# GPUs/goVideoCompressor

Hardware: AMD Instinct MI355X
Metric: encoded frames/sec (whole node), 1080p30->H.264 CRF23 (higher is better)
Workload: dtype uint8 (8-bit 4:2:0 samples, int32 transforms)

## Files before the change

csrc/kernels/bindings_hip.cc:

```cpp
#include <pybind11/pybind11.h>
#include <pybind11/stl.h>

#include <cstdint>
#include <stdexcept>
#include <vector>

#include "../common/hevc_ctu_coder.h"
#include "hevc_decode.h"
#include "route.h"

namespace py = pybind11;

extern "C" {
long long mivc_hevc_entropy_state_bytes(int W, int H);
int mivc_launch_hevc_entropy(const void* pic, int B, const int* qp, const void* ctu, const void* cu, const void* col,
                             const unsigned long long* nzmap, const int16_t* cy, const int16_t* cb, const int16_t* cr,
                             uint8_t* state, long long state_bytes, uint8_t* out, unsigned cap, unsigned* sizes,
                             int* errs, unsigned long long* offs, unsigned long long* offs_host, uint8_t* dst,
                             unsigned long long dst_cap, int* overflow, void* stream, unsigned long long* prof,
                             int* gprog, void* gctx);
int mivc_launch_hevc_decode(const mivc::gpu::HevcDecParams* p, int stage, void* stream);
void mivc_launch_synth(void* y, void* u, void* v, int width, int height, int slots, int frames, int frame0,
                       uint32_t seed, int bit_depth, int slot0, void* stream, int kind);
void mivc_launch_prep(const uint8_t* in_y, const uint8_t* in_u, const uint8_t* in_v, int w, int h,
                      int64_t in_stride_y, int64_t in_stride_c, int nframes, uint8_t* out_y, uint8_t* out_u,
                      uint8_t* out_v, int ow, int oh, int W, int H, void* stream, const int* fsel);
void mivc_launch_rgb_to_i420(const uint8_t* rgb, int w, int h, int nframes, uint8_t* y, uint8_t* u, uint8_t* v,
                             void* stream);
void mivc_launch_me(int B, int wmb, int hmb, const uint8_t* src_y, const uint8_t* ref_y, const int16_t* pred_mv,
                    int16_t* out_mv, int* out_cost, uint8_t* out_pred, int* out_intra_cost, const int* qp, int range,
                    int subpel, uint8_t* hp, const int8_t* aq, int planes_ready, int early_sad, void* stream,
                    const int* gate_cost, int gate_thresh, const int16_t* cost_mv, const void* route, int nbuf,
                    int role, int want, const int16_t* seed_mv);
void mivc_launch_me_ref_select(int B, int wmb, int hmb, int nref, int16_t* mv, int16_t* mv8, int* cost, uint8_t* pred,
                               const int16_t* xmv, const int* xcost, const uint8_t* xpred, int8_t* mref, const int* qp,
                               const int8_t* aq, void* stream, const void* route);
void mivc_launch_b_spatial(int B, int wmb, int hmb, void* hdr, const void* col, const uint8_t* src, const uint8_t* ref1,
                           const uint8_t* hp1, const uint8_t* const* ref0k, const uint8_t* const* hp0k, const int* w1,
                           int nref, uint8_t* pred_out, int* err, void* stream, const int* intra_cost, int* cost,
                           const int* qp, const int8_t* aq, int bias, const void* route, int nbuf);
void mivc_launch_b_direct(int B, int wmb, int hmb, const void* col, const int* dsf, const int* direct_copy, int nref,
                          int16_t* dmv, int8_t* dref, int16_t* pm0, int16_t* pm1, void* stream, const void* route,
                          int nbuf, uint8_t* czero, const int8_t* cmap);
void mivc_launch_b_spatial_exact(int B, int wmb, int hmb, void* hdr, const int* intra_cost, const int* cost,
                                 const uint8_t* czero, uint8_t* fix, void* stream, const void* route, int slice_rows,
                                 int tol);
void mivc_launch_b_spatial_fixup(int B, int wmb, int hmb, const void* hdr, const uint8_t* fix, const uint8_t* ref0,
                                 const uint8_t* hp0, const uint8_t* ref1, const uint8_t* hp1, uint8_t* pred_out,
                                 void* stream, const void* route, int nbuf);
void mivc_launch_p_refine(int B, int wmb, int hmb, const uint8_t* src_y, const uint8_t* ref, const uint8_t* hp,
                          const int16_t* mv_in, int16_t* mv_out, int* cost, const int16_t* pm, uint8_t* pred,
                          const int* qp, const int8_t* aq, void* stream, const void* route, int nbuf,
                          const uint8_t* chg_in, uint8_t* chg_out);
void mivc_launch_b_decide(int B, int wmb, int hmb, const uint8_t* src_y, const uint8_t* ref0, const uint8_t* ref1,
                          const uint8_t* hp0, const uint8_t* hp1, const int16_t* mv0, const int16_t* mv1,
                          const int* cost0, const int* cost1, const uint8_t* pred0, const uint8_t* pred1,
                          const int16_t* pm0, const int16_t* pm1, const int16_t* dmv, const int* qp, const int8_t* aq,
                          void* hdr, uint8_t* pred_out, int* cost_out, void* stream, const int* w1, int nref,
                          const int8_t* dref, const uint8_t* const* ref0k, const uint8_t* const* hp0k,
                          int direct_only, int bparts, int have_direct, int spatial, int dbias, const void* route,
                          int nbuf, const uint8_t* czero);
void mivc_launch_aq_offsets(int B, int wmb, int hmb, const uint8_t* sy, const uint8_t* su, const uint8_t* sv,
                            float strength, const float* extra, long long extra_stride, int8_t* out, void* stream,
                            const void* route);
void mivc_launch_mbtree(int B, int F, int lbw, int lbh, const int* blk_cost, const int* blk_mv, void* prop,
                        float strength, float* out, void* stream);
// ... 143 lines not shown
}

PYBIND11_MODULE(_hip, m) {
  m.doc() = "govideocompressor_amd gfx950 kernels (raw-pointer launch shims)";
  m.attr("arch") = "gfx950";
  m.def("route_bytes", []() { return static_cast<int>(sizeof(mivc::gpu::SlotRoute)); });

  m.def("synth", [](uintptr_t y, uintptr_t u, uintptr_t v, int w, int h, int slots, int frames, int frame0,
                    uint32_t seed, uintptr_t stream, int bit_depth, int slot0, int kind) {
    if (bit_depth != 8 && bit_depth != 10) throw std::invalid_argument("synth: bit_depth must be 8 or 10");
    if (kind < 0 || kind > 6) throw std::invalid_argument("synth: content kind 0..6");
    mivc_launch_synth(P<void>(y), P<void>(u), P<void>(v), w, h, slots, frames, frame0, seed, bit_depth, slot0,
                      S(stream), kind);
  }, py::arg("y"), py::arg("u"), py::arg("v"), py::arg("w"), py::arg("h"), py::arg("slots"), py::arg("frames"),
     py::arg("frame0"), py::arg("seed"), py::arg("stream"), py::arg("bit_depth") = 8, py::arg("slot0") = 0,
     py::arg("kind") = 0);
  m.def("prep", [](uintptr_t iy, uintptr_t iu, uintptr_t iv, int w, int h, int64_t sy, int64_t sc, int n,
                   uintptr_t oy, uintptr_t ou, uintptr_t ov, int ow, int oh, int W, int H, uintptr_t stream,
                   uintptr_t fsel) {
    if (ow != w || oh != h) throw std::invalid_argument("prep: resample with ops.scale (scale.hip) first");
    if (W < w || H < h || w < 2 || h < 2) throw std::invalid_argument("prep: bad geometry");
    mivc_launch_prep(P<uint8_t>(iy), P<uint8_t>(iu), P<uint8_t>(iv), w, h, sy, sc, n, P<uint8_t>(oy), P<uint8_t>(ou),
                     P<uint8_t>(ov), ow, oh, W, H, S(stream), P<int>(fsel));
  }, py::arg("iy"), py::arg("iu"), py::arg("iv"), py::arg("w"), py::arg("h"), py::arg("sy"), py::arg("sc"), py::arg("n"),
     py::arg("oy"), py::arg("ou"), py::arg("ov"), py::arg("ow"), py::arg("oh"), py::arg("W"), py::arg("H"),
     py::arg("stream"), py::arg("fsel") = 0);
  m.def("rgb_to_i420", [](uintptr_t rgb, int w, int h, int n, uintptr_t y, uintptr_t u, uintptr_t v,
                          uintptr_t stream) {
    mivc_launch_rgb_to_i420(P<uint8_t>(rgb), w, h, n, P<uint8_t>(y), P<uint8_t>(u), P<uint8_t>(v), S(stream));
  });
  m.def("me", [](int B, int wmb, int hmb, uintptr_t src, uintptr_t ref, uintptr_t pred_mv, uintptr_t out_mv,
                 uintptr_t out_cost, uintptr_t out_pred, uintptr_t out_intra, uintptr_t qp, int range, int subpel,
                 uintptr_t stream, uintptr_t hp, uintptr_t aq, int planes_ready, int early_sad, uintptr_t gate_cost,
                 int gate_thresh, uintptr_t cost_mv, uintptr_t route, int nbuf, int role, int want, uintptr_t seed_mv) {
    if (planes_ready && !hp) throw std::invalid_argument("me: planes_ready needs the hp buffer");
    if (route && (nbuf < 1 || role < 0 || role > 4 || (want != 0 && want != 1) || !planes_ready))
      throw std::invalid_argument("me: a routed search needs nbuf, a role (list-0 0..3 / list-1 4), want P/B and the planes");
    mivc_launch_me(B, wmb, hmb, P<uint8_t>(src), P<uint8_t>(ref), P<int16_t>(pred_mv), P<int16_t>(out_mv),
                   P<int>(out_cost), P<uint8_t>(out_pred), P<int>(out_intra), P<int>(qp), range, subpel,
                   P<uint8_t>(hp), P<int8_t>(aq), planes_ready, early_sad, S(stream), P<int>(gate_cost), gate_thresh,
                   P<int16_t>(cost_mv), P<void>(route), nbuf, role, want, P<int16_t>(seed_mv));
  }, py::arg("B"), py::arg("wmb"), py::arg("hmb"), py::arg("src"), py::arg("ref"), py::arg("pred_mv"),
     py::arg("out_mv"), py::arg("out_cost"), py::arg("out_pred"), py::arg("out_intra"), py::arg("qp"),
     py::arg("range"), py::arg("subpel"), py::arg("stream"), py::arg("hp") = 0, py::arg("aq") = 0,
     py::arg("planes_ready") = 0, py::arg("early_sad") = 0, py::arg("gate_cost") = 0, py::arg("gate_thresh") = 0,
     py::arg("cost_mv") = 0, py::arg("route") = 0, py::arg("nbuf") = 0, py::arg("role") = 0, py::arg("want") = 0,
     py::arg("seed_mv") = 0);
  m.def("me_ref_select", [](int B, int wmb, int hmb, int nref, uintptr_t mv, uintptr_t mv8, uintptr_t cost,
                            uintptr_t pred, uintptr_t xmv, uintptr_t xcost, uintptr_t xpred, uintptr_t mref,
                            uintptr_t qp, uintptr_t aq, uintptr_t stream, uintptr_t route) {
    if (nref < 2 || nref > 4) throw std::invalid_argument("me_ref_select: nref in 2..4");
    mivc_launch_me_ref_select(B, wmb, hmb, nref, P<int16_t>(mv), P<int16_t>(mv8), P<int>(cost), P<uint8_t>(pred),
                              P<int16_t>(xmv), P<int>(xcost), P<uint8_t>(xpred), P<int8_t>(mref), P<int>(qp),
                              P<int8_t>(aq), S(stream), P<void>(route));
  }, py::arg("B"), py::arg("wmb"), py::arg("hmb"), py::arg("nref"), py::arg("mv"), py::arg("mv8"), py::arg("cost"),
     py::arg("pred"), py::arg("xmv"), py::arg("xcost"), py::arg("xpred"), py::arg("mref"), py::arg("qp"), py::arg("aq"),
     py::arg("stream"), py::arg("route") = 0);
  m.def("b_spatial", [](int B, int wmb, int hmb, uintptr_t hdr, uintptr_t col, uintptr_t src, uintptr_t ref1,
                        uintptr_t hp1, std::vector<uintptr_t> ref0k, std::vector<uintptr_t> hp0k, std::vector<int> w1,
                        uintptr_t pred_out, uintptr_t err, uintptr_t stream, uintptr_t intra_cost, uintptr_t cost,
                        uintptr_t qp, uintptr_t aq, int bias, uintptr_t route, int nbuf) {
    const size_t n = ref0k.size();
    if (n < 1 || n > 4 || hp0k.size() != n || w1.size() != n)
      throw std::invalid_argument("b_spatial: 1..4 list-0 pictures with planes and weights");
    if (hmb > 272 || wmb > 480) throw std::invalid_argument("b_spatial: at most 272 MB rows and 480 columns");
    const uint8_t* rk[4];
    const uint8_t* hk[4];
    for (size_t i = 0; i < n; ++i) {
      rk[i] = P<uint8_t>(ref0k[i]);
      hk[i] = P<uint8_t>(hp0k[i]);
    }
    mivc_launch_b_spatial(B, wmb, hmb, P<void>(hdr), P<void>(col), P<uint8_t>(src), P<uint8_t>(ref1), P<uint8_t>(hp1),
                          rk, hk, w1.data(), static_cast<int>(n), P<uint8_t>(pred_out), P<int>(err), S(stream),
                          P<int>(intra_cost), P<int>(cost), P<int>(qp), P<int8_t>(aq), bias, P<void>(route), nbuf);
  }, py::arg("B"), py::arg("wmb"), py::arg("hmb"), py::arg("hdr"), py::arg("col"), py::arg("src"), py::arg("ref1"),
     py::arg("hp1"), py::arg("ref0k"), py::arg("hp0k"), py::arg("w1"), py::arg("pred_out"), py::arg("err"),
     py::arg("stream"), py::arg("intra_cost"), py::arg("cost"), py::arg("qp"), py::arg("aq"), py::arg("bias"),
     py::arg("route") = 0, py::arg("nbuf") = 0);
  m.def("b_direct", [](int B, int wmb, int hmb, uintptr_t col, std::vector<int> dsf, std::vector<int> direct_copy,
                       uintptr_t dmv, uintptr_t pm0, uintptr_t pm1, uintptr_t stream, uintptr_t dref, uintptr_t route,
// ... 587 lines not shown
```

csrc/kernels/me.hip:

```cpp
#include "me_search.h"

#include <cstdio>
#include <cstdlib>

namespace mivc {
namespace gpu {

constexpr int kHpRows = 8;

__device__ __forceinline__ void hp_load_row(const uint8_t* fr, int W, int H, int y, int x0, bool xin, int* p) {
  const uint8_t* row = fr + static_cast<size_t>(clampi(y, 0, H - 1)) * W;
  if (xin) {
    const uint32_t w0 = *reinterpret_cast<const uint32_t*>(row + x0 - 4);
    const uint32_t w1 = *reinterpret_cast<const uint32_t*>(row + x0);
    const uint32_t w2 = *reinterpret_cast<const uint32_t*>(row + x0 + 4);
    p[0] = __builtin_amdgcn_ubfe(w0, 16, 8);
    p[1] = __builtin_amdgcn_ubfe(w0, 24, 8);
#pragma unroll
    for (int k = 0; k < 4; ++k) p[2 + k] = __builtin_amdgcn_ubfe(w1, 8 * k, 8);
#pragma unroll
    for (int k = 0; k < 3; ++k) p[6 + k] = __builtin_amdgcn_ubfe(w2, 8 * k, 8);
  } else {
#pragma unroll
    for (int c = 0; c < 9; ++c) p[c] = row[clampi(x0 - 2 + c, 0, W - 1)];
// ... 112 lines not shown
  while (win) {
    const int i = __builtin_ctzll(win);
    win &= win - 1;
    const size_t o = o0 + i;
    const size_t xo = (__builtin_amdgcn_readlane(bk, i) - 1) * plane + o;
    reinterpret_cast<uint32_t*>(a.pred + o * 256)[lane] = reinterpret_cast<const uint32_t*>(a.xpred + xo * 256)[lane];
  }
}

#ifdef MIVC_ME_PROFILE
extern "C" void mivc_me_prof_read(unsigned long long* out) {
  hipMemcpyFromSymbol(out, HIP_SYMBOL(g_me_prof), sizeof(unsigned long long) * 64 * 12);
}
#endif

}
}

using namespace mivc::gpu;

extern "C" void mivc_launch_me_halfpel(int B, int W, int H, const uint8_t* ref_y, uint8_t* hp, void* stream,
                                       const void* route, int nbuf) {
  const int PW = W + 2 * kHpMargin, PH = H + 2 * kHpMargin;
  const dim3 grid((PW / 4 + 63) / 64, (PH + 4 * kHpRows - 1) / (4 * kHpRows), B);
  hipLaunchKernelGGL(me_halfpel_planes, grid, dim3(256), 0, static_cast<hipStream_t>(stream), ref_y, W, H, hp,
                     static_cast<const SlotRoute*>(route), nbuf);
}

extern "C" void mivc_launch_me(int B, int wmb, int hmb, const uint8_t* src_y, const uint8_t* ref_y,
                               const int16_t* pred_mv, int16_t* out_mv, int* out_cost, uint8_t* out_pred,
                               int* out_intra_cost, const int* qp, int range, int subpel, uint8_t* hp_buf,
                               const int8_t* aq, int planes_ready, int early_sad, void* stream,
                               const int* gate_cost, int gate_thresh, const int16_t* cost_mv, const void* route,
                               int nbuf, int role, int want, const int16_t* seed_mv) {
  hipStream_t s = static_cast<hipStream_t>(stream);
  const int W = wmb * 16, H = hmb * 16;
  uint8_t* hp = hp_buf;
  if (!hp) {
    const size_t hp_bytes = static_cast<size_t>(B) * 3 * (W + 2 * kHpMargin) * (H + 2 * kHpMargin) + 64;
    keep_async_pool();
    if (hipMallocAsync(reinterpret_cast<void**>(&hp), hp_bytes, s) != hipSuccess) {
      fprintf(stderr, "mivc_launch_me: hipMallocAsync(%zu) failed\n", hp_bytes);
      abort();
    }
  }
  if (route && !(planes_ready && hp_buf)) {
    fprintf(stderr, "mivc_launch_me: a routed search needs the resident half-sample pool\n");
    abort();
  }
  if (!(planes_ready && hp_buf)) mivc_launch_me_halfpel(B, W, H, ref_y, hp, stream, nullptr, 0);
  MeArgs a;
  a.g = Geom{B, wmb, hmb, W, H};
  a.src_y = src_y;
  a.ref_y = ref_y;
  a.pred_mv = pred_mv;
  a.out_mv = out_mv;
  a.out_cost = out_cost;
  a.out_pred = out_pred;
  a.out_intra_cost = out_intra_cost;
  a.qp = qp;
  a.range = range < kMaxR ? range : kMaxR;
  a.subpel = subpel;
  a.hp = hp;
  a.aq = aq;
  a.early_sad = early_sad;
  a.gate_cost = gate_cost;
  a.gate_thresh = gate_thresh;
  a.cost_mv = cost_mv;
  a.rt = static_cast<const SlotRoute*>(route);
  a.nbuf = nbuf;
  a.role = role;
  a.want = want;
  a.seed_mv = seed_mv;
  if (gate_cost) launch_me_gated(a, s);
  else if (a.range <= 8) hipLaunchKernelGGL((me_p16x16<8, 1>), dim3(wmb * hmb, B), dim3(64), 0, s, a);
  else hipLaunchKernelGGL((me_p16x16<kMaxR, 1>), dim3(wmb * hmb, B), dim3(64), 0, s, a);
  if (!hp_buf) (void)hipFreeAsync(hp, s);
}

extern "C" void mivc_launch_me_ref_select(int B, int wmb, int hmb, int nref, int16_t* mv, int16_t* mv8, int* cost,
                                          uint8_t* pred, const int16_t* xmv, const int* xcost, const uint8_t* xpred,
                                          int8_t* mref, const int* qp, const int8_t* aq, void* stream,
                                          const void* route) {
  RefSelArgs a;
  a.rt = static_cast<const SlotRoute*>(route);
  a.g = Geom{B, wmb, hmb, wmb * 16, hmb * 16};
  a.nref = nref;
  a.mv = mv;
  a.mv8 = mv8;
  a.cost = cost;
  a.pred = pred;
  a.xmv = xmv;
  a.xcost = xcost;
  a.xpred = xpred;
  a.mref = mref;
  a.qp = qp;
  a.aq = aq;
  hipLaunchKernelGGL(me_ref_select, dim3((wmb * hmb + 63) / 64, B), dim3(64), 0, static_cast<hipStream_t>(stream), a);
}
```

csrc/kernels/me_gated.hip:

```cpp
#define MIVC_ME_GATED_UNIT
#include "me_search.h"

namespace mivc {
namespace gpu {

void launch_me_gated(const MeArgs& a, hipStream_t s) {
  const dim3 grid((a.g.nmb() + kGateSpan - 1) / kGateSpan, a.g.B);
  if (a.range <= 8) hipLaunchKernelGGL((me_p16x16<8, kGateSpan>), grid, dim3(64), 0, s, a);
  else hipLaunchKernelGGL((me_p16x16<kMaxR, kGateSpan>), grid, dim3(64), 0, s, a);
}

}
}
```

csrc/kernels/me_search.h:

```cpp
#pragma once
#include "kcommon.h"
#include "qpel.h"

namespace mivc {
namespace gpu {

struct MeArgs {
  Geom g;
  const uint8_t* src_y;
  const uint8_t* ref_y;
  const int16_t* pred_mv;
  int16_t* out_mv;
  int* out_cost;
  uint8_t* out_pred;
  int* out_intra_cost;
  const int* qp;
  int range;
  int subpel;
  const uint8_t* hp;
  const int8_t* aq;
  int early_sad;
  const int* gate_cost;
  int gate_thresh;
  const int16_t* cost_mv;
// ... 125 lines not shown
    }
  }
  int best = 0x7FFFFFFF;
#pragma unroll
  for (int j = 0; j < DYN; ++j) {
    const int dy = dy0 + j;
    const int mvx = (cx + dx - R) * 4, mvy = (cy + dy - R) * 4;
    const int cost = static_cast<int>(acc[j]) + lambda * (mvbits_se(mvx - pmx) + mvbits_se(mvy - pmy));
    const int key = (g < G && dy < side) ? ((cost << 12) | (dy * side + dx)) : 0x7FFFFFFF;
    best = key < best ? key : best;
  }
  return best;
}

#if defined(MIVC_ME_PROFILE) && !defined(MIVC_ME_GATED_UNIT)
__device__ unsigned long long g_me_prof[64][12];
#define MPROF(ph) do { if (lin < 64 && lane == 0) g_me_prof[lin][ph] = clock64(); } while (0)
#else
#define MPROF(ph) do {} while (0)
#endif

typedef float v4f __attribute__((ext_vector_type(4)));
typedef _Float16 v4h __attribute__((ext_vector_type(4)));

__device__ __forceinline__ v4h me_neg_h16(int lane) {
  const int mg = lane >> 4, mn = lane & 15;
  v4h negH;
#pragma unroll
  for (int j = 0; j < 4; ++j) negH[j] = (__builtin_popcount(mn & (4 * mg + j)) & 1) ? _Float16(1.0f) : _Float16(-1.0f);
  return negH;
}

template <int MAXR, int SPAN>
__device__ __forceinline__ void me_mb(const MeArgs a, int slot_run, int mb_run, int lambda_run, bool first,
                                      v4h negH_hoisted) {
  const Geom& g = a.g;
  const int nmb = g.nmb();
  int lin = 0, slot = slot_run, mb = mb_run;
  if constexpr (SPAN == 1) {
    const int total = nmb * g.B;
    lin = blockIdx.y * gridDim.x + blockIdx.x;
    if ((total & 7) == 0) lin = (lin & 7) * (total >> 3) + (lin >> 3);
    slot = lin / nmb;
    mb = lin - slot * nmb;
  }
  const int mx = mb % g.wmb, my = mb / g.wmb;
  int lane = threadIdx.x;
  if constexpr (SPAN > 1) asm volatile("" : "+v"(lane));
  const int X0 = mx * 16, Y0 = my * 16;
  if constexpr (SPAN == 1) {
    if (a.rt) {
      const SlotRoute& rr = a.rt[slot];
      if (rr.kind != a.want || (a.role < RO_L1 && a.role >= rr.n0)) return;
    }
  }
  const size_t rslot = route_index(a.rt, a.nbuf, slot, a.role);
  const uint8_t* src = a.src_y + slot * g.ysize();
  const uint8_t* ref = a.ref_y + rslot * g.ysize();
  const int W = g.W, H = g.H;
  int lambda = lambda_run;
  if constexpr (SPAN == 1) {
    const int qp = clampi(a.qp[slot] + (a.aq ? a.aq[static_cast<size_t>(slot) * nmb + mb] : 0), 0, 51);
    lambda = h264::kLambda[qp];
  }
  const int R = a.range < MAXR ? a.range : MAXR;

  __shared__ MeShared<MAXR> S;
  if constexpr (SPAN == 1) {
    if (a.gate_cost) {
      const size_t og = static_cast<size_t>(slot) * nmb + mb;
      const int thr = a.gate_thresh >= 0 ? a.gate_thresh : -a.gate_thresh * lambda;
      if (a.gate_cost[og] <= thr) {
        if (lane == 0) {
          a.out_cost[og] = kNoCost;
          if (a.out_intra_cost) a.out_intra_cost[og] = kNoCost;
        }
        return;
      }
    }
  }
  (void)lin;

  MPROF(0);
  const int r4 = lane >> 2, c4 = (lane & 3) * 4;
  const uint32_t my_src = *reinterpret_cast<const uint32_t*>(src + static_cast<size_t>(Y0 + r4) * W + X0 + c4);
  int nbv = 0;
  if (lane < 16) nbv = my > 0 ? src[static_cast<size_t>(Y0 - 1) * W + X0 + lane] : 0;
  else if (lane < 32) nbv = mx > 0 ? src[static_cast<size_t>(Y0 + lane - 16) * W + X0 - 1] : 0;
  else if (lane == 32) nbv = (mx > 0 && my > 0) ? src[static_cast<size_t>(Y0 - 1) * W + X0 - 1] : 0;
  int pmx = 0, pmy = 0;
  int cand_x[6] = {0, 0, 0, 0, 0, 0}, cand_y[6] = {0, 0, 0, 0, 0, 0};
  if (a.seed_mv) {
    const size_t so = (static_cast<size_t>(slot) * nmb + mb) * 2;
    cand_x[5] = (a.seed_mv[so] + 2) >> 2;
    cand_y[5] = (a.seed_mv[so + 1] + 2) >> 2;
  }
  if (a.pred_mv) {
// ... 289 lines not shown
        int cost = s + lambda * (mvbits_se(mvx - pmx) + mvbits_se(mvy - pmy));
        int key = (cost << 4) | ci;
        qkey = key < qkey ? key : qkey;
      }
      qkey = wave_min_key(qkey);
      best_cost = qkey >> 4;
      int qx, qy;
      ring(qkey & 15, 1, &qx, &qy);
      hx += qx;
      hy += qy;
    }
    MPROF(6);
    best_mvx += hx;
    best_mvy += hy;
  }
  const size_t o = static_cast<size_t>(slot) * nmb + mb;
  MPROF(7);
  {
    int dqx = best_mvx - 4 * bx, dqy = best_mvy - 4 * by;
    int q = (dqy & 3) * 4 + (dqx & 3), ox = dqx >> 2, oy = dqy >> 2;
    int offa = S.qoff[2 * q], offb = S.qoff[2 * q + 1];
    reinterpret_cast<uint32_t*>(a.out_pred + o * 256)[lane] = pred4(c4 + ox + 2, r4 + oy + 2, offa, offb);
  }
  MPROF(8);
  if (lane == 0) {
    a.out_mv[o * 2] = static_cast<int16_t>(best_mvx);
    a.out_mv[o * 2 + 1] = static_cast<int16_t>(best_mvy);
    a.out_cost[o] = best_cost;
    if (a.out_intra_cost) a.out_intra_cost[o] = intra_key + lambda * 4;
  }
  MPROF(9);
}

constexpr int kGateSpan = 8;
constexpr int kGateWaves = 6;

template <int MAXR, int SPAN>
__global__ __launch_bounds__(64) __attribute__((amdgpu_waves_per_eu(SPAN == 1 ? 8 : kGateWaves, 8))) void me_p16x16(MeArgs a) {
  if constexpr (SPAN == 1) {
    me_mb<MAXR, 1>(a, 0, 0, 0, true, v4h{});
  } else {
    const Geom& g = a.g;
    const int nmb = g.nmb();
    const int lane = threadIdx.x;
    const int nruns = gridDim.x;
    const int total = nruns * g.B;
    int lin = blockIdx.y * gridDim.x + blockIdx.x;
    if ((total & 7) == 0) lin = (lin & 7) * (total >> 3) + (lin >> 3);
    const int slot = lin / nruns, mb0 = (lin - slot * nruns) * SPAN;
    if (a.rt) {
      const SlotRoute& rr = a.rt[slot];
      if (rr.kind != a.want || (a.role < RO_L1 && a.role >= rr.n0)) return;
    }
    int lam = 0;
    bool search = false;
    if (lane < SPAN && mb0 + lane < nmb) {
      const size_t og = static_cast<size_t>(slot) * nmb + mb0 + lane;
      const int qp = clampi(a.qp[slot] + (a.aq ? a.aq[og] : 0), 0, 51);
      lam = h264::kLambda[qp];
      search = true;
      if (a.gate_cost) {
        const int thr = a.gate_thresh >= 0 ? a.gate_thresh : -a.gate_thresh * lam;
        if (a.gate_cost[og] <= thr) {
          search = false;
          a.out_cost[og] = kNoCost;
          if (a.out_intra_cost) a.out_intra_cost[og] = kNoCost;
        }
      }
    }
    unsigned long long mask = __ballot(search);
    if (!mask) return;
    const v4h negH = me_neg_h16(lane);
    bool first = true;
    while (mask) {
      const int i = __builtin_ctzll(mask);
      mask &= mask - 1;
      wave_sync();
      me_mb<MAXR, SPAN>(a, slot, mb0 + i, __builtin_amdgcn_readlane(lam, i), first, negH);
      first = false;
    }
  }
}

void launch_me_gated(const MeArgs& a, hipStream_t s);

}
}
```

govideocompressor_amd/models/h264_gpu.py:

```python
from __future__ import annotations

import concurrent.futures as cf
import math
import os
import time
from dataclasses import dataclass

import numpy as np
import torch

from ..ops import native
from .gop import PicPlan, col_to_list0, dpb_frames, fixed_types, gop_plan, h264_plan

MB_HDR_BYTES = 64
NO_COST = 0x3FFFFFFF
ROUTE_DTYPE = np.dtype([("kind", "i1"), ("cur", "i1"), ("n0", "i1"), ("l1", "i1"), ("l0", "i1", (4,)),
                        ("w1", "<i2", (4,)), ("dsf", "<i2", (4,)), ("dcopy", "i1", (4,)), ("flags", "u1"),
                        ("col_l1", "i1"), ("disp", "<i2")])
assert ROUTE_DTYPE.itemsize == 32
COL_NONE = -128


def col_map_row(cur: PicPlan, col: PicPlan) -> np.ndarray:
    return np.array([[COL_NONE if m is None else m - r for r, m in enumerate(row)] for row in col_to_list0(cur, col)],
# ... 258 lines not shown
                    torch.zeros((B, H // 2, W // 2), dtype=u8, device=dev))

        self.src = planes()
        self.nb = params.eff_bframes()
        self.nref = params.eff_refs()
        self.nref_frames = dpb_frames(self.nref, params.eff_pyramid(), self.nb)
        self.nbuf = self.nref_frames + 2
        NB = self.nbuf
        self.rec_pool = (torch.zeros((B, NB, H, W), dtype=u8, device=dev),
                         torch.zeros((B, NB, H // 2, W // 2), dtype=u8, device=dev),
                         torch.zeros((B, NB, H // 2, W // 2), dtype=u8, device=dev))
        self.rec = [tuple(p[:, i] for p in self.rec_pool) for i in range(NB)]
        self.hp_bytes = 3 * (H + 8) * (W + 8)
        self.hp_pool = torch.empty(B * NB * self.hp_bytes + 64, dtype=u8, device=dev)
        self.hdr = [torch.zeros((B, nmb, MB_HDR_BYTES), dtype=u8, device=dev) for _ in range(2)]
        self.coef = [torch.zeros((B, nmb, COEF_PER_MB), dtype=i16, device=dev) for _ in range(2)]
        self.nz = torch.zeros((B, nmb, 16), dtype=u8, device=dev)
        self.mv = torch.zeros((B, nmb, 2), dtype=i16, device=dev)
        self.mv_tmp = torch.zeros((B, nmb, 2), dtype=i16, device=dev)
        self.mv8 = torch.zeros((B, nmb, 4, 2), dtype=i16, device=dev)
        self.prev_mv = torch.zeros((B, nmb, 2), dtype=i16, device=dev)
        self.me_cost = torch.zeros((B, nmb), dtype=i32, device=dev)
        self.intra_cost = torch.zeros((B, nmb), dtype=i32, device=dev)
        self.pred = torch.zeros((B, nmb, 256), dtype=u8, device=dev)
        self.mref = torch.zeros((B, nmb), dtype=torch.int8, device=dev)
        self.dref = torch.zeros((B, nmb, 4), dtype=torch.int8, device=dev)
        self.seed = [torch.zeros((B, nmb, 2), dtype=i16, device=dev) for _ in range(2)]
        self._slot_ar = torch.arange(B, device=dev)
        if self.nref > 1:
            K = self.nref - 1
            self.xmv = torch.zeros((K, B, nmb, 2), dtype=i16, device=dev)
            self.xcost = torch.zeros((K, B, nmb), dtype=i32, device=dev)
            self.xpred = torch.zeros((K, B, nmb, 256), dtype=u8, device=dev)
            self.xpm = torch.zeros((B, nmb, 2), dtype=i16, device=dev)
        if self.nb:
            self.mv1 = torch.zeros((B, nmb, 2), dtype=i16, device=dev)
            self.me_cost1 = torch.zeros((B, nmb), dtype=i32, device=dev)
            self.pred1 = torch.zeros((B, nmb, 256), dtype=u8, device=dev)
            self.pred_b = torch.zeros((B, nmb, 256), dtype=u8, device=dev)
            self.cost_b = torch.zeros((B, nmb), dtype=i32, device=dev)
            self.pm0 = torch.zeros((B, nmb, 2), dtype=i16, device=dev)
            self.pm1 = torch.zeros((B, nmb, 2), dtype=i16, device=dev)
            self.dmv = torch.zeros((B, nmb, 16), dtype=i16, device=dev)
            self.czero = torch.zeros((B, nmb), dtype=u8, device=dev)
            self.sfix = torch.zeros((B, nmb), dtype=u8, device=dev)
            self.col_pool = torch.zeros((B, NB, nmb, MB_HDR_BYTES), dtype=u8, device=dev)
        if params.eff_weightp():
            self.src_me = torch.zeros((B, H, W), dtype=u8, device=dev)
        self.intra_flag = torch.zeros((B, nmb), dtype=u8, device=dev)
        self.aq = torch.zeros((B, nmb), dtype=torch.int8, device=dev)
        if self.aq_auto:
            self.aq_terms = torch.zeros((B, nmb), dtype=torch.float32, device=dev)
        self.qp_flags = torch.zeros((B, nmb), dtype=u8, device=dev)
        self.qp_pre = torch.zeros((B, nmb), dtype=u8, device=dev)
        self.intra_count = torch.zeros((B,), dtype=i32, device=dev)
        self.qp = torch.zeros((B,), dtype=i32, device=dev)
        self.err_bufs = [torch.zeros((1,), dtype=i32, device=dev) for _ in range(2)]
        self.err = self.err_bufs[0]
        self.h_err = [torch.zeros((1,), dtype=i32).pin_memory() for _ in range(2)]
        self._batch_no = 0
        self._ring_last: list = [None, None]
        self._inflight: list = []
        self.p_intra_mbs = torch.zeros((), dtype=torch.int64, device=dev)
        self.far_ref_mbs = torch.zeros((), dtype=torch.int64, device=dev)
        self.sfix_mbs = torch.zeros((), dtype=torch.int64, device=dev)
        self.sconv_mbs = torch.zeros((), dtype=torch.int64, device=dev)
        self.una_mbs = torch.zeros((), dtype=torch.int64, device=dev)
# ... 184 lines not shown
                seed1 = P(self.seed[1])
        if st["P"]:
            sy_me, wp = sy, 0
            if st["wp"] is not None:
                wp = st["wp"].data_ptr()
                with stt("weightp"):
                    self.hip.wp_src(sy, P(self.src_me), st["wp_src"].data_ptr(), B, self.H * self.W, s)
                sy_me = P(self.src_me)
            with stt("me_p"):
                self.hip.me(B, wmb, hmb, sy_me, py, P(self.prev_mv), P(self.mv), P(self.me_cost), P(self.pred),
                            P(self.intra_cost), P(self.qp), self.p.me_range, self.p.subpel, s, hpp, aq, 1,
                            self.p.p_early_sad, 0, 0, 0, rt, NB, 0, SK["P"], seed0)
                if getattr(self, "_chg", None) is None:
                    self._chg = [torch.zeros((B, self.nmb), dtype=torch.uint8, device=self.dev) for _ in range(2)]
                for it in range(int(self.p.skip_refine)):
                    a_, b_ = (self.mv, self.mv_tmp) if it % 2 == 0 else (self.mv_tmp, self.mv)
                    self.hip.p_refine(B, wmb, hmb, sy_me, py, hpp, P(a_), P(b_), P(self.me_cost), P(self.prev_mv),
                                      P(self.pred), P(self.qp), aq, s, rt, NB,
                                      0 if (it == 0 or not self.p.refine_skip) else P(self._chg[(it - 1) % 2]),
                                      P(self._chg[it % 2]) if self.p.refine_skip else 0)
                if int(self.p.skip_refine) % 2:
                    self.mv.copy_(torch.where(st["pmask"][:, None, None], self.mv_tmp, self.mv))
            mv8 = 0
            if self.p.eff_partitions():
                with stt("part"):
                    self.hip.p_part8(B, wmb, hmb, sy_me, py, hpp, P(self.mv), P(self.prev_mv), P(self.me_cost),
                                     P(self.pred), P(self.mv8), P(self.qp), aq, int(self.p.part_overhead),
                                     int(self.p.part_min_satd), s, rt, NB)
                mv8 = P(self.mv8)
            self.prev_mv.copy_(torch.where(st["pmask"][:, None, None], self.mv, self.prev_mv))
            nr = st["maxn0"]
            if nr > 1:
                with stt("me_ref"):
                    for k in range(1, nr):
                        self.xpm.copy_((self.mv.float() * st["xscale"][k - 1][:, None, None]).round_().clamp_(-2048, 2047))
                        self.hip.me(B, wmb, hmb, sy, py, P(self.xpm), P(self.xmv[k - 1]), P(self.xcost[k - 1]),
                                    P(self.xpred[k - 1]), 0, P(self.qp), int(self.p.ref_range), self.p.subpel, s,
                                    hpp, aq, 1, self.p.p_early_sad, P(self.me_cost), self._ref_gate(),
                                    P(self.prev_mv), rt, NB, k, SK["P"])
                    self.hip.me_ref_select(B, wmb, hmb, nr, P(self.mv), mv8, P(self.me_cost), P(self.pred),
                                           P(self.xmv), P(self.xcost), P(self.xpred), P(self.mref), P(self.qp), aq,
                                           s, rt)
                    self.far_ref_mbs += ((self.mref > 0) & st["pmask"][:, None]).sum()
            else:
                self.mref.zero_()
            if cut is not None:
                self.intra_cost.masked_fill_(cut[:, None], -1)
            with stt("inter"):
                self.hip.encode_inter(B, wmb, hmb, sy, su, sv, py, pu, pv, py, pu, pv, P(self.pred), P(self.mv),
                                      P(self.me_cost), P(self.intra_cost), P(self.qp), cqo, P(hdr), P(coef),
                                      P(self.nz), P(self.intra_flag), P(self.intra_count), s, aq,
                                      t8=int(self.p.eff_t8x8()), mv8=mv8, mref=P(self.mref), wp=wp,
                                      trellis=int(self.p.trellis), trellis_lambda=float(self.p.trellis_lambda),
                                      route=rt, nbuf=NB, **pre)
        if st["B"]:
            br = self.p.b_me_range
            spatial = self.p.direct == "spatial"
            sfast = spatial and not self.p.spatial_wavefront
            mode = 2 if sfast else int(spatial)
            bg = int(self.p.b_gate) if (not spatial or sfast or self.p.spatial_gate) else 0
            dbias = int(self.p.tdirect_bias) if not spatial else (int(self.p.direct_bias) if sfast else 0)
            with stt("me_b"):
                self.hip.b_direct(B, wmb, hmb, P(self.col_pool), [0], [1], P(self.dmv), P(self.pm0), P(self.pm1), s,
                                  P(self.dref), rt, NB, P(self.czero), st["cmap"])
                if self._una_count:
                    self.una_mbs += ((self.dref < 0).any(dim=2) & st["bmask"][:, None]).sum()
                if bg != 0 or sfast:
                    self.hip.b_decide(B, wmb, hmb, sy, py, py, hpp, hpp, P(self.mv), P(self.mv1), P(self.me_cost),
                                      P(self.me_cost1), P(self.pred), P(self.pred1), P(self.pm0), P(self.pm1),
                                      P(self.dmv), P(self.qp), aq, P(hdr), P(self.pred_b), P(self.cost_b), s, [32],
                                      P(self.dref), [], [], 1, spatial=mode, route=rt, nbuf=NB, czero=P(self.czero))
                gate = P(self.cost_b) if bg != 0 else 0
                self.hip.me(B, wmb, hmb, sy, py, P(self.pm0), P(self.mv), P(self.me_cost), P(self.pred),
                            P(self.intra_cost), P(self.qp), br, self.p.subpel, s, hpp, aq, 1, self.p.b_early_sad,
                            gate, bg, 0, rt, NB, 0, SK["B"], seed0)
                self.hip.me(B, wmb, hmb, sy, py, P(self.pm1), P(self.mv1), P(self.me_cost1), P(self.pred1), 0,
                            P(self.qp), br, self.p.subpel, s, hpp, aq, 1, self.p.b_early_sad, gate, bg, 0, rt, NB,
                            4, SK["B"], seed1)
            with stt("b_decide"):
                self.hip.b_decide(B, wmb, hmb, sy, py, py, hpp, hpp, P(self.mv), P(self.mv1), P(self.me_cost),
                                  P(self.me_cost1), P(self.pred), P(self.pred1), P(self.pm0), P(self.pm1),
                                  P(self.dmv), P(self.qp), aq, P(hdr), P(self.pred_b), P(self.cost_b), s, [32],
                                  P(self.dref), [], [], 0, int(self.p.eff_partitions() and self.p.bpartitions),
                                  int(bg != 0 or sfast), mode, dbias, route=rt, nbuf=NB, czero=P(self.czero))
            if sfast:
                with stt("b_spatial"):
                    self.hip.b_spatial_exact(B, wmb, hmb, P(hdr), P(self.intra_cost), P(self.cost_b), P(self.czero),
                                             P(self.sfix), s, rt, self.slice_rows, int(self.p.spatial_fix_tol))
                    self.sfix_mbs += (self.sfix == 1).sum()
                    self.sconv_mbs += (self.sfix == 2).sum()
                    self.hip.b_spatial_fixup(B, wmb, hmb, P(hdr), P(self.sfix), py, hpp, py, hpp, P(self.pred_b), s,
                                             rt, NB)
            elif spatial:
                with stt("b_spatial"):
                    self.hip.b_spatial(B, wmb, hmb, P(hdr), P(self.col_pool), sy, py, hpp, [py], [hpp], [32],
                                       P(self.pred_b), P(self.err), s, P(self.intra_cost), P(self.cost_b), P(self.qp),
                                       aq, int(self.p.direct_bias), rt, NB)
            with stt("inter"):
                self.hip.encode_inter(B, wmb, hmb, sy, su, sv, py, pu, pv, py, pu, pv, P(self.pred_b), P(self.mv),
                                      P(self.cost_b), P(self.intra_cost), P(self.qp), cqo, P(hdr), P(coef),
                                      P(self.nz), P(self.intra_flag), P(self.intra_count), s, aq, pu, pv, 1,
                                      int(self.p.eff_t8x8()), 0, [32], [], [], 0, 0, int(self.p.trellis),
                                      float(self.p.trellis_lambda), rt, NB, **pre)
        if inter:
            self.p_intra_mbs += self.intra_count.sum()
            flag_ptr, count_ptr = P(self.intra_flag), P(self.intra_count)
        else:
            self.prev_mv.zero_()
            flag_ptr, count_ptr = 0, 0
        trial = not inter or self.p.i4x4_in_p or cut is not None
        if getattr(self, "_intra_prog", None) is None:
# ... 838 lines not shown
```

Before: 16940.

## Compact gated ME survivors into a list and fuse multi-reference/B-side searches

Replaces the span-based gated motion search, where each wave scanned 8 MBs and idled on gated-off ones, with two kernels. The first does a ballot and atomic compaction of surviving macroblocks into a global list. The second is a persistent-style kernel that walks that list across up to three sides (reference lists or L0/L1) in one launch. This aims to cut wasted wave launches on skipped MBs and the per-reference launch overhead for multi-ref P and bidirectional B search. In exchange it adds a compaction pass, a memset and a list buffer. Survivor ordering changes, which may hurt cache locality of reference reads.

```diff
diff --git a/csrc/kernels/bindings_hip.cc b/csrc/kernels/bindings_hip.cc
--- a/csrc/kernels/bindings_hip.cc
+++ b/csrc/kernels/bindings_hip.cc
@@ -3,6 +3,7 @@
 
 #include <cstdint>
 #include <stdexcept>
+#include <tuple>
 #include <vector>
 
 #include "../common/hevc_ctu_coder.h"
@@ -31,7 +32,23 @@
                     int16_t* out_mv, int* out_cost, uint8_t* out_pred, int* out_intra_cost, const int* qp, int range,
                     int subpel, uint8_t* hp, const int8_t* aq, int planes_ready, int early_sad, void* stream,
                     const int* gate_cost, int gate_thresh, const int16_t* cost_mv, const void* route, int nbuf,
-                    int role, int want, const int16_t* seed_mv);
+                    int role, int want, const int16_t* seed_mv, uint32_t* gate_list);
+struct MivcMeSide {
+  const uint8_t* ref_y;
+  const uint8_t* hp;
+  const int16_t* pred_mv;
+  const int16_t* cost_mv;
+  const int16_t* seed_mv;
+  int16_t* out_mv;
+  int* out_cost;
+  uint8_t* out_pred;
+  int* out_intra_cost;
+  int role;
+};
+void mivc_launch_me_gated_multi(int B, int wmb, int hmb, const uint8_t* src_y, const int* qp, int range, int subpel,
+                                const int8_t* aq, int early_sad, const int* gate_cost, int gate_thresh,
+                                const void* route, int nbuf, int want, uint32_t* list, int max_groups, int nsides,
+                                const MivcMeSide* sides, int gate_only, void* stream);
 void mivc_launch_me_ref_select(int B, int wmb, int hmb, int nref, int16_t* mv, int16_t* mv8, int* cost, uint8_t* pred,
                                const int16_t* xmv, const int* xcost, const uint8_t* xpred, int8_t* mref, const int* qp,
                                const int8_t* aq, void* stream, const void* route);
@@ -241,20 +258,56 @@
   m.def("me", [](int B, int wmb, int hmb, uintptr_t src, uintptr_t ref, uintptr_t pred_mv, uintptr_t out_mv,
                  uintptr_t out_cost, uintptr_t out_pred, uintptr_t out_intra, uintptr_t qp, int range, int subpel,
                  uintptr_t stream, uintptr_t hp, uintptr_t aq, int planes_ready, int early_sad, uintptr_t gate_cost,
-                 int gate_thresh, uintptr_t cost_mv, uintptr_t route, int nbuf, int role, int want, uintptr_t seed_mv) {
+                 int gate_thresh, uintptr_t cost_mv, uintptr_t route, int nbuf, int role, int want, uintptr_t seed_mv,
+                 uintptr_t gate_list, int64_t gate_list_words) {
     if (planes_ready && !hp) throw std::invalid_argument("me: planes_ready needs the hp buffer");
+    if (gate_list && gate_list_words < 2 + static_cast<int64_t>(B) * wmb * hmb)
+      throw std::invalid_argument("me: gate_list needs 2 + B * nmb words");
     if (route && (nbuf < 1 || role < 0 || role > 4 || (want != 0 && want != 1) || !planes_ready))
       throw std::invalid_argument("me: a routed search needs nbuf, a role (list-0 0..3 / list-1 4), want P/B and the planes");
     mivc_launch_me(B, wmb, hmb, P<uint8_t>(src), P<uint8_t>(ref), P<int16_t>(pred_mv), P<int16_t>(out_mv),
                    P<int>(out_cost), P<uint8_t>(out_pred), P<int>(out_intra), P<int>(qp), range, subpel,
                    P<uint8_t>(hp), P<int8_t>(aq), planes_ready, early_sad, S(stream), P<int>(gate_cost), gate_thresh,
-                   P<int16_t>(cost_mv), P<void>(route), nbuf, role, want, P<int16_t>(seed_mv));
+                   P<int16_t>(cost_mv), P<void>(route), nbuf, role, want, P<int16_t>(seed_mv),
+                   P<uint32_t>(gate_list));
   }, py::arg("B"), py::arg("wmb"), py::arg("hmb"), py::arg("src"), py::arg("ref"), py::arg("pred_mv"),
      py::arg("out_mv"), py::arg("out_cost"), py::arg("out_pred"), py::arg("out_intra"), py::arg("qp"),
      py::arg("range"), py::arg("subpel"), py::arg("stream"), py::arg("hp") = 0, py::arg("aq") = 0,
      py::arg("planes_ready") = 0, py::arg("early_sad") = 0, py::arg("gate_cost") = 0, py::arg("gate_thresh") = 0,
      py::arg("cost_mv") = 0, py::arg("route") = 0, py::arg("nbuf") = 0, py::arg("role") = 0, py::arg("want") = 0,
-     py::arg("seed_mv") = 0);
+     py::arg("seed_mv") = 0, py::arg("gate_list") = 0, py::arg("gate_list_words") = 0);
+  m.def("me_gated_multi", [](int B, int wmb, int hmb, uintptr_t src, uintptr_t qp, int range, int subpel,
+                             uintptr_t stream, uintptr_t aq, int early_sad, uintptr_t gate_cost, int gate_thresh,
+                             uintptr_t route, int nbuf, int want,
+                             const std::vector<std::tuple<uintptr_t, uintptr_t, uintptr_t, uintptr_t, uintptr_t, uintptr_t,
+                                                          uintptr_t, uintptr_t, uintptr_t, int>>& sides,
+                             uintptr_t list, int64_t list_words, int max_groups, int gate_only) {
+    if (B < 1 || wmb < 1 || hmb < 1 || static_cast<int64_t>(B) * wmb * hmb > 0x3FFFFFFF)
+      throw std::invalid_argument("me_gated_multi: bad geometry");
+    if (!gate_cost) throw std::invalid_argument("me_gated_multi: needs gate_cost");
+    if (sides.empty() || sides.size() > 3) throw std::invalid_argument("me_gated_multi: 1..3 sides");
+    if (list && list_words < 2 + static_cast<int64_t>(B) * wmb * hmb)
+      throw std::invalid_argument("me_gated_multi: list needs 2 + B * nmb words");
+    if (route && (nbuf < 1 || (want != 0 && want != 1)))
+      throw std::invalid_argument("me_gated_multi: a routed search needs nbuf and want P/B");
+    MivcMeSide sd[3];
+    for (size_t k = 0; k < sides.size(); ++k) {
+      const auto& t = sides[k];
+      sd[k] = MivcMeSide{P<uint8_t>(std::get<0>(t)), P<uint8_t>(std::get<1>(t)), P<int16_t>(std::get<2>(t)),
+                         P<int16_t>(std::get<3>(t)), P<int16_t>(std::get<4>(t)), P<int16_t>(std::get<5>(t)),
+                         P<int>(std::get<6>(t)),     P<uint8_t>(std::get<7>(t)), P<int>(std::get<8>(t)),
+                         std::get<9>(t)};
+      if (!sd[k].ref_y || !sd[k].hp || !sd[k].out_mv || !sd[k].out_cost || !sd[k].out_pred)
+        throw std::invalid_argument("me_gated_multi: a side needs ref, hp (planes built), out_mv, out_cost and out_pred");
+      if (sd[k].role < 0 || sd[k].role > 4) throw std::invalid_argument("me_gated_multi: role list-0 0..3 / list-1 4");
+    }
+    mivc_launch_me_gated_multi(B, wmb, hmb, P<uint8_t>(src), P<int>(qp), range, subpel, P<int8_t>(aq), early_sad,
+                               P<int>(gate_cost), gate_thresh, P<void>(route), nbuf, want, P<uint32_t>(list), max_groups,
+                               static_cast<int>(sides.size()), sd, gate_only, S(stream));
+  }, py::arg("B"), py::arg("wmb"), py::arg("hmb"), py::arg("src"), py::arg("qp"), py::arg("range"), py::arg("subpel"),
+     py::arg("stream"), py::arg("aq"), py::arg("early_sad"), py::arg("gate_cost"), py::arg("gate_thresh"),
+     py::arg("route"), py::arg("nbuf"), py::arg("want"), py::arg("sides"), py::arg("list") = 0,
+     py::arg("list_words") = 0, py::arg("max_groups") = 0, py::arg("gate_only") = 0);
   m.def("me_ref_select", [](int B, int wmb, int hmb, int nref, uintptr_t mv, uintptr_t mv8, uintptr_t cost,
                             uintptr_t pred, uintptr_t xmv, uintptr_t xcost, uintptr_t xpred, uintptr_t mref,
                             uintptr_t qp, uintptr_t aq, uintptr_t stream, uintptr_t route) {
diff --git a/csrc/kernels/me.hip b/csrc/kernels/me.hip
--- a/csrc/kernels/me.hip
+++ b/csrc/kernels/me.hip
@@ -168,7 +168,7 @@
                                int* out_intra_cost, const int* qp, int range, int subpel, uint8_t* hp_buf,
                                const int8_t* aq, int planes_ready, int early_sad, void* stream,
                                const int* gate_cost, int gate_thresh, const int16_t* cost_mv, const void* route,
-                               int nbuf, int role, int want, const int16_t* seed_mv) {
+                               int nbuf, int role, int want, const int16_t* seed_mv, uint32_t* gate_list) {
   hipStream_t s = static_cast<hipStream_t>(stream);
   const int W = wmb * 16, H = hmb * 16;
   uint8_t* hp = hp_buf;
@@ -208,8 +208,13 @@
   a.role = role;
   a.want = want;
   a.seed_mv = seed_mv;
-  if (gate_cost) launch_me_gated(a, s);
-  else if (a.range <= 8) hipLaunchKernelGGL((me_p16x16<8, 1>), dim3(wmb * hmb, B), dim3(64), 0, s, a);
+  if (gate_cost) {
+    MeListArgs l = {};
+    l.a = a;
+    l.nsides = 1;
+    l.side[0] = MeSide{ref_y, hp, pred_mv, cost_mv, seed_mv, out_mv, out_cost, out_pred, out_intra_cost, role};
+    launch_me_list(l, gate_list, 0, false, s);
+  } else if (a.range <= 8) hipLaunchKernelGGL((me_p16x16<8, 1>), dim3(wmb * hmb, B), dim3(64), 0, s, a);
   else hipLaunchKernelGGL((me_p16x16<kMaxR, 1>), dim3(wmb * hmb, B), dim3(64), 0, s, a);
   if (!hp_buf) (void)hipFreeAsync(hp, s);
 }
diff --git a/csrc/kernels/me_gated.hip b/csrc/kernels/me_gated.hip
--- a/csrc/kernels/me_gated.hip
+++ b/csrc/kernels/me_gated.hip
@@ -1,14 +1,194 @@
 #define MIVC_ME_GATED_UNIT
 #include "me_search.h"
+
+#include <cstdio>
+#include <cstdlib>
 
 namespace mivc {
 namespace gpu {
 
-void launch_me_gated(const MeArgs& a, hipStream_t s) {
-  const dim3 grid((a.g.nmb() + kGateSpan - 1) / kGateSpan, a.g.B);
-  if (a.range <= 8) hipLaunchKernelGGL((me_p16x16<8, kGateSpan>), grid, dim3(64), 0, s, a);
-  else hipLaunchKernelGGL((me_p16x16<kMaxR, kGateSpan>), grid, dim3(64), 0, s, a);
+constexpr int kGateBlock = 1024;
+constexpr int kGatePer = 4;
+
+__device__ __forceinline__ bool side_live(const SlotRoute* rt, int slot, int role) {
+  return !rt || !(role < RO_L1 && role >= rt[slot].n0);
+}
+
+__global__ __launch_bounds__(kGateBlock) void me_gate_list(MeListArgs l) {
+  const MeArgs& a = l.a;
+  const int nmb = a.g.nmb();
+  const uint32_t total = static_cast<uint32_t>(nmb) * a.g.B;
+  const int lane = threadIdx.x & 63, wave = threadIdx.x >> 6;
+  __shared__ uint32_t wave_n[kGateBlock / 64];
+  __shared__ uint32_t base_s;
+  unsigned long long mask[kGatePer];
+  uint32_t mine = 0;
+#pragma unroll
+  for (int r = 0; r < kGatePer; ++r) {
+    const uint32_t og = (blockIdx.x * kGatePer + r) * kGateBlock + threadIdx.x;
+    bool search = false;
+    if (og < total) {
+      const int slot = og / nmb;
+      if (!a.rt || a.rt[slot].kind == a.want) {
+        const int qp = clampi(a.qp[slot] + (a.aq ? a.aq[og] : 0), 0, 51);
+        const int lam = h264::kLambda[qp];
+        const int thr = a.gate_thresh >= 0 ? a.gate_thresh : -a.gate_thresh * lam;
+        const bool gated = a.gate_cost[og] <= thr;
+        bool any = false;
+#pragma unroll
+        for (int k = 0; k < kMaxSides; ++k) {
+          if (k >= l.nsides || !side_live(a.rt, slot, l.side[k].role)) continue;
+          any = true;
+          if (gated) {
+            l.side[k].out_cost[og] = kNoCost;
+            if (l.side[k].out_intra_cost) l.side[k].out_intra_cost[og] = kNoCost;
+          }
+        }
+        search = any && !gated;
+      }
+    }
+    mask[r] = __ballot(search);
+    mine += __builtin_popcountll(mask[r]);
+  }
+  if (lane == 0) wave_n[wave] = mine;
+  __syncthreads();
+  if (threadIdx.x == 0) {
+    uint32_t n = 0;
+#pragma unroll
+    for (int w = 0; w < kGateBlock / 64; ++w) n += wave_n[w];
+    base_s = n ? atomicAdd(&l.list[0], n) : 0u;
+  }
+  __syncthreads();
+  uint32_t pos = base_s;
+  for (int w = 0; w < wave; ++w) pos += wave_n[w];
+#pragma unroll
+  for (int r = 0; r < kGatePer; ++r) {
+    if ((mask[r] >> lane) & 1)
+      l.list[2 + pos + __builtin_popcountll(mask[r] & ((1ull << lane) - 1))] = (blockIdx.x * kGatePer + r) * kGateBlock + threadIdx.x;
+    pos += __builtin_popcountll(mask[r]);
+  }
+}
+
+template <int MAXR>
+__global__ __launch_bounds__(64) __attribute__((amdgpu_waves_per_eu(kGateWaves, 8))) void me_search_list(MeListArgs l) {
+  const uint32_t nsides = l.nsides;
+  const uint32_t nitems = l.list[0] * nsides;
+  uint32_t it = blockIdx.x, end = nitems, step = gridDim.x;
+  if ((gridDim.x & 7) == 0) {
+    const uint32_t x = blockIdx.x & 7;
+    step = gridDim.x >> 3;
+    it = static_cast<uint32_t>(static_cast<uint64_t>(nitems) * x >> 3) + (blockIdx.x >> 3);
+    end = static_cast<uint32_t>(static_cast<uint64_t>(nitems) * (x + 1) >> 3);
+  }
+  if (it >= end) return;
+  const int nmb = l.a.g.nmb();
+  const v4h negH = me_neg_h16(threadIdx.x);
+  bool first = true;
+  uint32_t og = l.list[2 + it / nsides];
+  for (;;) {
+    const uint32_t k = it % nsides;
+    og = __builtin_amdgcn_readfirstlane(og);
+    const int slot = og / nmb, mb = og - slot * nmb;
+    it += step;
+    uint32_t og_next = 0;
+    if (it < end) og_next = l.list[2 + it / nsides];
+    const MeSide& sd = l.side[k];
+    if (side_live(l.a.rt, slot, sd.role)) {
+      MeArgs a = l.a;
+      a.ref_y = sd.ref_y;
+      a.hp = sd.hp;
+      a.pred_mv = sd.pred_mv;
+      a.cost_mv = sd.cost_mv;
+      a.seed_mv = sd.seed_mv;
+      a.out_mv = sd.out_mv;
+      a.out_cost = sd.out_cost;
+      a.out_pred = sd.out_pred;
+      a.out_intra_cost = sd.out_intra_cost;
+      a.role = sd.role;
+      wave_sync();
+      me_mb<MAXR, 2>(a, slot, mb, first, negH);
+      first = false;
+    }
+    if (it >= end) break;
+    og = og_next;
+  }
+}
+
+constexpr int kSearchGroups = 256 * 4 * kGateWaves;
+
+void launch_me_list(const MeListArgs& args, uint32_t* list, int max_groups, bool gate_only, hipStream_t s) {
+  MeListArgs l = args;
+  const size_t total = static_cast<size_t>(l.a.g.nmb()) * l.a.g.B;
+  if (!l.a.gate_cost || l.nsides < 1 || l.nsides > kMaxSides || total == 0 || total > 0x3FFFFFFFu) {
+    fprintf(stderr, "launch_me_list: needs a gate, 1..%d sides and fewer than 2^30 MBs\n", kMaxSides);
+    abort();
+  }
+  l.list = list;
+  if (!list) {
+    keep_async_pool();
+    if (hipMallocAsync(reinterpret_cast<void**>(&l.list), (total + 2) * sizeof(uint32_t), s) != hipSuccess) {
+      fprintf(stderr, "launch_me_list: hipMallocAsync(%zu) failed\n", (total + 2) * sizeof(uint32_t));
+      abort();
+    }
+  }
+  (void)hipMemsetAsync(l.list, 0, 2 * sizeof(uint32_t), s);
+  hipLaunchKernelGGL(me_gate_list, dim3(static_cast<unsigned>((total + kGateBlock * kGatePer - 1) / (kGateBlock * kGatePer))),
+                     dim3(kGateBlock), 0, s, l);
+  if (!gate_only) {
+    int groups = kSearchGroups;
+    if (max_groups > 0 && max_groups < groups) groups = max_groups;
+    if (l.a.range <= 8) hipLaunchKernelGGL((me_search_list<8>), dim3(groups), dim3(64), 0, s, l);
+    else hipLaunchKernelGGL((me_search_list<kMaxR>), dim3(groups), dim3(64), 0, s, l);
+  }
+  if (!list) (void)hipFreeAsync(l.list, s);
 }
 
 }
 }
+
+using namespace mivc::gpu;
+
+struct MivcMeSide {
+  const uint8_t* ref_y;
+  const uint8_t* hp;
+  const int16_t* pred_mv;
+  const int16_t* cost_mv;
+  const int16_t* seed_mv;
+  int16_t* out_mv;
+  int* out_cost;
+  uint8_t* out_pred;
+  int* out_intra_cost;
+  int role;
+};
+static_assert(sizeof(MivcMeSide) == sizeof(MeSide), "MivcMeSide mirrors MeSide");
+
+extern "C" void mivc_launch_me_gated_multi(int B, int wmb, int hmb, const uint8_t* src_y, const int* qp, int range,
+                                           int subpel, const int8_t* aq, int early_sad, const int* gate_cost,
+                                           int gate_thresh, const void* route, int nbuf, int want, uint32_t* list,
+                                           int max_groups, int nsides, const MivcMeSide* sides, int gate_only,
+                                           void* stream) {
+  if (nsides < 1 || nsides > kMaxSides) {
+    fprintf(stderr, "mivc_launch_me_gated_multi: 1..%d sides\n", kMaxSides);
+    abort();
+  }
+  MeListArgs l = {};
+  l.a.g = Geom{B, wmb, hmb, wmb * 16, hmb * 16};
+  l.a.src_y = src_y;
+  l.a.qp = qp;
+  l.a.range = range < kMaxR ? range : kMaxR;
+  l.a.subpel = subpel;
+  l.a.aq = aq;
+  l.a.early_sad = early_sad;
+  l.a.gate_cost = gate_cost;
+  l.a.gate_thresh = gate_thresh;
+  l.a.rt = static_cast<const SlotRoute*>(route);
+  l.a.nbuf = nbuf;
+  l.a.want = want;
+  l.nsides = nsides;
+  for (int k = 0; k < nsides; ++k) {
+    const MivcMeSide& m = sides[k];
+    l.side[k] = MeSide{m.ref_y, m.hp, m.pred_mv, m.cost_mv, m.seed_mv, m.out_mv, m.out_cost, m.out_pred,
+                       m.out_intra_cost, m.role};
+  }
+  launch_me_list(l, list, max_groups, gate_only != 0, static_cast<hipStream_t>(stream));
+}
diff --git a/csrc/kernels/me_search.h b/csrc/kernels/me_search.h
--- a/csrc/kernels/me_search.h
+++ b/csrc/kernels/me_search.h
@@ -181,8 +181,7 @@
 }
 
 template <int MAXR, int SPAN>
-__device__ __forceinline__ void me_mb(const MeArgs a, int slot_run, int mb_run, int lambda_run, bool first,
-                                      v4h negH_hoisted) {
+__device__ __forceinline__ void me_mb(const MeArgs a, int slot_run, int mb_run, bool first, v4h negH_hoisted) {
   const Geom& g = a.g;
   const int nmb = g.nmb();
   int lin = 0, slot = slot_run, mb = mb_run;
@@ -207,11 +206,8 @@
   const uint8_t* src = a.src_y + slot * g.ysize();
   const uint8_t* ref = a.ref_y + rslot * g.ysize();
   const int W = g.W, H = g.H;
-  int lambda = lambda_run;
-  if constexpr (SPAN == 1) {
-    const int qp = clampi(a.qp[slot] + (a.aq ? a.aq[static_cast<size_t>(slot) * nmb + mb] : 0), 0, 51);
-    lambda = h264::kLambda[qp];
-  }
+  const int qp = clampi(a.qp[slot] + (a.aq ? a.aq[static_cast<size_t>(slot) * nmb + mb] : 0), 0, 51);
+  const int lambda = h264::kLambda[qp];
   const int R = a.range < MAXR ? a.range : MAXR;
 
   __shared__ MeShared<MAXR> S;
@@ -567,57 +563,37 @@
   MPROF(9);
 }
 
-constexpr int kGateSpan = 8;
 constexpr int kGateWaves = 6;
 
 template <int MAXR, int SPAN>
-__global__ __launch_bounds__(64) __attribute__((amdgpu_waves_per_eu(SPAN == 1 ? 8 : kGateWaves, 8))) void me_p16x16(MeArgs a) {
-  if constexpr (SPAN == 1) {
-    me_mb<MAXR, 1>(a, 0, 0, 0, true, v4h{});
-  } else {
-    const Geom& g = a.g;
-    const int nmb = g.nmb();
-    const int lane = threadIdx.x;
-    const int nruns = gridDim.x;
-    const int total = nruns * g.B;
-    int lin = blockIdx.y * gridDim.x + blockIdx.x;
-    if ((total & 7) == 0) lin = (lin & 7) * (total >> 3) + (lin >> 3);
-    const int slot = lin / nruns, mb0 = (lin - slot * nruns) * SPAN;
-    if (a.rt) {
-      const SlotRoute& rr = a.rt[slot];
-      if (rr.kind != a.want || (a.role < RO_L1 && a.role >= rr.n0)) return;
-    }
-    int lam = 0;
-    bool search = false;
-    if (lane < SPAN && mb0 + lane < nmb) {
-      const size_t og = static_cast<size_t>(slot) * nmb + mb0 + lane;
-      const int qp = clampi(a.qp[slot] + (a.aq ? a.aq[og] : 0), 0, 51);
-      lam = h264::kLambda[qp];
-      search = true;
-      if (a.gate_cost) {
-        const int thr = a.gate_thresh >= 0 ? a.gate_thresh : -a.gate_thresh * lam;
-        if (a.gate_cost[og] <= thr) {
-          search = false;
-          a.out_cost[og] = kNoCost;
-          if (a.out_intra_cost) a.out_intra_cost[og] = kNoCost;
-        }
-      }
-    }
-    unsigned long long mask = __ballot(search);
-    if (!mask) return;
-    const v4h negH = me_neg_h16(lane);
-    bool first = true;
-    while (mask) {
-      const int i = __builtin_ctzll(mask);
-      mask &= mask - 1;
-      wave_sync();
-      me_mb<MAXR, SPAN>(a, slot, mb0 + i, __builtin_amdgcn_readlane(lam, i), first, negH);
-      first = false;
-    }
-  }
-}
-
-void launch_me_gated(const MeArgs& a, hipStream_t s);
-
-}
-}
+__global__ __launch_bounds__(64) __attribute__((amdgpu_waves_per_eu(8, 8))) void me_p16x16(MeArgs a) {
+  static_assert(SPAN == 1, "gated launches go through the survivor list (me_gated.hip)");
+  me_mb<MAXR, 1>(a, 0, 0, true, v4h{});
+}
+
+constexpr int kMaxSides = 3;
+
+struct MeSide {
+  const uint8_t* ref_y;
+  const uint8_t* hp;
+  const int16_t* pred_mv;
+  const int16_t* cost_mv;
+  const int16_t* seed_mv;
+  int16_t* out_mv;
+  int* out_cost;
+  uint8_t* out_pred;
+  int* out_intra_cost;
+  int role;
+};
+
+struct MeListArgs {
+  MeArgs a;
+  MeSide side[kMaxSides];
+  int nsides;
+  uint32_t* list;
+};
+
+void launch_me_list(const MeListArgs& l, uint32_t* list, int max_groups, bool gate_only, hipStream_t s);
+
+}
+}
diff --git a/govideocompressor_amd/models/h264_gpu.py b/govideocompressor_amd/models/h264_gpu.py
--- a/govideocompressor_amd/models/h264_gpu.py
+++ b/govideocompressor_amd/models/h264_gpu.py
@@ -314,7 +314,8 @@
             self.xmv = torch.zeros((K, B, nmb, 2), dtype=i16, device=dev)
             self.xcost = torch.zeros((K, B, nmb), dtype=i32, device=dev)
             self.xpred = torch.zeros((K, B, nmb, 256), dtype=u8, device=dev)
-            self.xpm = torch.zeros((B, nmb, 2), dtype=i16, device=dev)
+            self.xpm = torch.zeros((K, B, nmb, 2), dtype=i16, device=dev)
+        self.gate_list = torch.zeros(B * nmb + 2, dtype=i32, device=dev)
         if self.nb:
             self.mv1 = torch.zeros((B, nmb, 2), dtype=i16, device=dev)
             self.me_cost1 = torch.zeros((B, nmb), dtype=i32, device=dev)
@@ -565,12 +566,21 @@
             nr = st["maxn0"]
             if nr > 1:
                 with stt("me_ref"):
+                    fused = hasattr(self.hip, "me_gated_multi")
                     for k in range(1, nr):
-                        self.xpm.copy_((self.mv.float() * st["xscale"][k - 1][:, None, None]).round_().clamp_(-2048, 2047))
-                        self.hip.me(B, wmb, hmb, sy, py, P(self.xpm), P(self.xmv[k - 1]), P(self.xcost[k - 1]),
-                                    P(self.xpred[k - 1]), 0, P(self.qp), int(self.p.ref_range), self.p.subpel, s,
-                                    hpp, aq, 1, self.p.p_early_sad, P(self.me_cost), self._ref_gate(),
-                                    P(self.prev_mv), rt, NB, k, SK["P"])
+                        self.xpm[k - 1].copy_((self.mv.float() * st["xscale"][k - 1][:, None, None]).round_().clamp_(-2048, 2047))
+                        if not fused:
+                            self.hip.me(B, wmb, hmb, sy, py, P(self.xpm[k - 1]), P(self.xmv[k - 1]), P(self.xcost[k - 1]),
+                                        P(self.xpred[k - 1]), 0, P(self.qp), int(self.p.ref_range), self.p.subpel, s,
+                                        hpp, aq, 1, self.p.p_early_sad, P(self.me_cost), self._ref_gate(),
+                                        P(self.prev_mv), rt, NB, k, SK["P"])
+                    if fused:
+                        self.hip.me_gated_multi(
+                            B, wmb, hmb, sy, P(self.qp), int(self.p.ref_range), self.p.subpel, s, aq,
+                            self.p.p_early_sad, P(self.me_cost), self._ref_gate(), rt, NB, SK["P"],
+                            [(py, hpp, P(self.xpm[k - 1]), P(self.prev_mv), 0, P(self.xmv[k - 1]), P(self.xcost[k - 1]),
+                              P(self.xpred[k - 1]), 0, k) for k in range(1, nr)],
+                            P(self.gate_list), self.gate_list.numel())
                     self.hip.me_ref_select(B, wmb, hmb, nr, P(self.mv), mv8, P(self.me_cost), P(self.pred),
                                            P(self.xmv), P(self.xcost), P(self.xpred), P(self.mref), P(self.qp), aq,
                                            s, rt)
@@ -604,12 +614,20 @@
                                       P(self.dmv), P(self.qp), aq, P(hdr), P(self.pred_b), P(self.cost_b), s, [32],
                                       P(self.dref), [], [], 1, spatial=mode, route=rt, nbuf=NB, czero=P(self.czero))
                 gate = P(self.cost_b) if bg != 0 else 0
-                self.hip.me(B, wmb, hmb, sy, py, P(self.pm0), P(self.mv), P(self.me_cost), P(self.pred),
-                            P(self.intra_cost), P(self.qp), br, self.p.subpel, s, hpp, aq, 1, self.p.b_early_sad,
-                            gate, bg, 0, rt, NB, 0, SK["B"], seed0)
-                self.hip.me(B, wmb, hmb, sy, py, P(self.pm1), P(self.mv1), P(self.me_cost1), P(self.pred1), 0,
-                            P(self.qp), br, self.p.subpel, s, hpp, aq, 1, self.p.b_early_sad, gate, bg, 0, rt, NB,
-                            4, SK["B"], seed1)
+                if gate and hasattr(self.hip, "me_gated_multi"):
+                    self.hip.me_gated_multi(
+                        B, wmb, hmb, sy, P(self.qp), br, self.p.subpel, s, aq, self.p.b_early_sad, gate, bg, rt, NB,
+                        SK["B"],
+                        [(py, hpp, P(self.pm0), 0, seed0, P(self.mv), P(self.me_cost), P(self.pred), P(self.intra_cost), 0),
+                         (py, hpp, P(self.pm1), 0, seed1, P(self.mv1), P(self.me_cost1), P(self.pred1), 0, 4)],
+                        P(self.gate_list), self.gate_list.numel())
+                else:
+                    self.hip.me(B, wmb, hmb, sy, py, P(self.pm0), P(self.mv), P(self.me_cost), P(self.pred),
+                                P(self.intra_cost), P(self.qp), br, self.p.subpel, s, hpp, aq, 1, self.p.b_early_sad,
+                                gate, bg, 0, rt, NB, 0, SK["B"], seed0)
+                    self.hip.me(B, wmb, hmb, sy, py, P(self.pm1), P(self.mv1), P(self.me_cost1), P(self.pred1), 0,
+                                P(self.qp), br, self.p.subpel, s, hpp, aq, 1, self.p.b_early_sad, gate, bg, 0, rt, NB,
+                                4, SK["B"], seed1)
             with stt("b_decide"):
                 self.hip.b_decide(B, wmb, hmb, sy, py, py, hpp, hpp, P(self.mv), P(self.mv1), P(self.me_cost),
                                   P(self.me_cost1), P(self.pred), P(self.pred1), P(self.pm0), P(self.pm1),
```

Result: no change. 17040, median of 6 (+0.6%).
